# jrl-umi3218/jrl-walkgen

Measured on AMD Instinct MI355X. Metric: QP-MPC ticks/sec (batch=4096, N=16), higher is better.
Workload: dtype f64

## Files before the change

### jrl-walkgen_amd/csrc/wg_capi.hip

```cpp
#include <hip/hip_runtime.h>

#include <climits>
#include <cmath>
#include <cstdarg>
#include <cstdio>
#include <cstdlib>
#include <cstring>
#include <limits>
#include <memory>
#include <mutex>
#include <string>
#include <type_traits>
#include <vector>

#include "../../include/wg_mpc.h"
#include "wg_ql_device.hpp"
#include "wg_tick_device.hpp"
#include "wg_tick_kernels.hpp"
#include "wg_pldp_device.hpp"
#include "wg_dimitrov_device.hpp"
#include "wg_preview_device.hpp"
#include "wg_gramian_device.hpp"
#include "wg_zmpdisc_device.hpp"
#include "wg_footcons_device.hpp"
// ... 562 lines not shown
  m->hip_l_lo = -30.0 / 180.0 * wg::kPi; m->hip_l_hi = 45.0 / 180.0 * wg::kPi;
  m->hip_r_lo = -30.0 / 180.0 * wg::kPi; m->hip_r_hi = 45.0 / 180.0 * wg::kPi;
  m->hip_vmax = 0.0; m->hip_amax = 0.1; m->feet_cross_max = 5.0 / 180.0 * wg::kPi;
  m->step_period = 0.8; m->ds_period = 1e9; m->dsss_period = 0.8;
  m->t_single = 0.7; m->t_double = 0.1; m->step_height = 0.05; m->feet_distance = 0.2;
}

void wg_gait_init(const wg_model_t *, wg_gait_state_t *s, const double com0[3], const double left_xyt[3],
                  const double right_xyt[3]) {
  memset(s, 0, sizeof *s);
  s->online = 1; s->time_to_stop = -1.0;
  for (int k = 0; k < 3; k++) {
    s->lf[k].x = left_xyt[0]; s->lf[k].y = left_xyt[1]; s->lf[k].theta = left_xyt[2];
    s->rf[k].x = right_xyt[0]; s->rf[k].y = right_xyt[1]; s->rf[k].theta = right_xyt[2];
  }
  s->phase = WG_DS; s->foot = WG_LEFT; s->time_limit = 1000000000; s->nb_steps_left = 1;
  s->sup_x = left_xyt[0]; s->sup_y = left_xyt[1]; s->sup_yaw = left_xyt[2] * wg::kPi / 180;
  s->com_x[0] = com0[0]; s->com_y[0] = com0[1]; s->com_z = com0[2];
  s->front_com_x[0] = com0[0]; s->front_com_y[0] = com0[1];
  s->nb_steps_ssds = 2; s->rot_support_foot = WG_LEFT;
}

int wg_mpc_configure_ctx(wg_ctx_t *ctx, const wg_model_t *model) {
  if (int rc = use_ctx(ctx)) return rc;
  if (!model) return fail(WG_ERR_BAD_ARG, "null model");
  if (model->N < 2 || model->N > wg::kNMaxH) return fail(WG_ERR_BAD_ARG, "N=%d outside [2,%d]", model->N, wg::kNMaxH);
  if ((int)(model->T / model->Tctrl) != WG_SAMPLES_PER_TICK)
    return fail(WG_ERR_BAD_ARG, "T/Tctrl must be %d", WG_SAMPLES_PER_TICK);
  if (tick_max_prw_steps(*model) > wg::kSMax)
    return fail(WG_ERR_BAD_ARG, "step_period=%g: a horizon of N=%d instants of T=%g previews up to %d steps, the tick holds %d",
                model->step_period, model->N, model->T, tick_max_prw_steps(*model), wg::kSMax);
  const size_t lds = TickPlan(*model).lds;
  if (lds > 160 * 1024) return fail(WG_ERR_TOO_LARGE, "tick needs %zu B of LDS > 160 KiB", lds);
  std::vector<double> qb;
  if (model->flags & (WG_FLAG_GRAMIAN_MFMA_F64 | WG_FLAG_GRAMIAN_MFMA_F32)) {
    qb.resize((size_t)model->N * model->N);
    const int prec = (model->flags & WG_FLAG_GRAMIAN_MFMA_F32) ? WG_GRAMIAN_F32 : WG_GRAMIAN_F64;
    if (int rc = wg_gramian_batch_ctx(ctx, 1, model->N, &model->T, &model->com_height_qp, model->alpha, model->beta, model->gamma,
                                  prec, qb.data()))
      return rc;
  }
  std::lock_guard<std::mutex> lk(ctx->mu);
  std::unique_ptr<wg::TickTables> host_tables_p(new wg::TickTables);
  wg::TickTables &host_tables = *host_tables_p;
  wg::build_tables(*model, host_tables, qb.empty() ? nullptr : qb.data());
  if (!host_tables.blocks_ok && !qb.empty())
    return fail(WG_ERR_BAD_ARG, "the matrix-core Gramian is not positive definite enough for ql0002's factorisation");
  if (const char *e = getenv("WG_QL_SUMS")) {
    const std::string v(e);
    if (v == "ordered") host_tables.ql_sums = wg::kSumsOrdered;
    else if (v == "doubt") host_tables.ql_sums = wg::kSumsDoubt;
    else if (!v.empty() && v != "guarded") return fail(WG_ERR_BAD_ARG, "WG_QL_SUMS=%s: ordered, doubt or unset", e);
  }
  if (!ctx->tables_dev) HIP_TRY(hipMalloc(reinterpret_cast<void **>(&ctx->tables_dev), sizeof(wg::TickTables)));
  if (!ctx->model_dev) HIP_TRY(hipMalloc(reinterpret_cast<void **>(&ctx->model_dev), sizeof(wg_model_t)));
  if (int rc = ctx_wait_own(ctx)) return rc;
  HostScope hs(ctx);
  WG_H2D(ctx->tables_dev, &host_tables, sizeof host_tables);
  WG_H2D(ctx->model_dev, model, sizeof(wg_model_t));
  WG_HOST_WAIT();
  ctx->model = *model;
  ctx->model_set = true;
  return WG_OK;
}

size_t wg_mpc_tick_lds_bytes_for(const wg_model_t *model) {
  if (!model || model->N < 2 || model->N > wg::kNMaxH || tick_max_prw_steps(*model) > wg::kSMax) return 0;
  return TickPlan(*model).lds;
}

size_t wg_mpc_tick_lds_bytes_ctx(wg_ctx_t *ctx) {
  if (!ctx || !ctx->model_set) return 0;
  return TickPlan(ctx->model).lds;
}

int wg_mpc_reserve_ctx(wg_ctx_t *ctx, int max_gaits) {
  if (int rc = use_ctx(ctx)) return rc;
  if (!ctx->model_set) return fail(WG_ERR_BAD_ARG, "wg_mpc_configure() has not been called on this context");
  if (max_gaits < 1) return fail(WG_ERR_BAD_ARG, "max_gaits = %d", max_gaits);
  const TickPlan plan(ctx->model);
  std::lock_guard<std::mutex> launch_lk(ctx->launch_mu);
  double *zs = nullptr;
  if (int rc = plan.reserve_slots(ctx, max_gaits, &zs)) return rc;
  return ctx->run_buf.reserve(run_buf_bytes(max_gaits));
}

}
namespace {
int tick_launch(wg_ctx_t *ctx, int B, wg_gait_state_t *states, wg_tick_out_t *outs, int *diag, int advance_calls, int *hist, int hist_cap, int *hist_len, void *hip_stream, wg_gait_state_t *host_states, int *host_done) {
  if (int rc = tick_check(ctx, B, states)) return rc;
  if (hist && (!hist_len || hist_cap <= 0)) return fail(WG_ERR_BAD_ARG, "hist needs hist_len and hist_cap > 0");
  if (B == 0) return WG_OK;
  const TickPlan plan(ctx->model);
  if (int rc = plan.raise_lds(WG_KERNEL_BY_VIEW(wg_mpc_tick_kernel, plan.view))) return rc;
  const int grid = B;
  hipStream_t st = reinterpret_cast<hipStream_t>(hip_stream);
  std::lock_guard<std::mutex> launch_lk(ctx->launch_mu);
  if (int rc = slot_claim(ctx, ctx->guard_order, st, "tick / run")) return rc;
  double *zs = nullptr;
  if (int rc = plan.reserve_slots(ctx, grid, &zs)) return rc;
  int *order = nullptr, *iters_out = nullptr;
  if (B > ctx->num_cu * plan.per_cu() && !host_states && env_flag("WG_TICK_LPT", true))
    if (int rc = lpt_prepare(ctx->tick_lpt, states, B, st, &order, &iters_out)) return rc;
  WG_LAUNCH_BY_VIEW(wg_mpc_tick_kernel, plan.view, grid, plan.launch_lds, st, B, ctx->model, ctx->tables_dev, states, outs, diag, advance_calls, hist,
                    hist_cap, hist_len, (unsigned)plan.qlb, zs, (unsigned)plan.zslot, plan.ecap, host_states, host_done, order, iters_out);
  HIP_TRY(hipGetLastError());
// ... 1350 lines not shown
```

### jrl-walkgen_amd/csrc/wg_prof.hpp

```cpp
#pragma once
#include <hip/hip_runtime.h>

namespace wg {

enum ProfSlot : int {
  PS_NORMS = 0, PS_DIAGCHK = 1, PS_CHOL = 2 , PS_INVERSE = 3,
  PS_RESID = 4, PS_ZTWW_RESID = 5, PS_XSHIFT = 6, PS_BACKSUB_RESID = 7, PS_XMAG_RESID = 8,
  PS_SCAN = 9, PS_FDIFF = 10, PS_NEWNORMAL = 11, PS_SWEEP = 12, PS_ROUTE = 13, PS_STEP_PRE = 14, PS_BACKSUB_STEP = 15,
  PS_PICKDROP = 16, PS_STEP = 17, PS_ADD = 18, PS_XMAG_ADD = 19, PS_TAIL = 20,
  PS_RESET_BODY = 24, PS_RESID_GRAD = 25, PS_RESID_FWD = 26, PS_RESID_GX = 27,
  PS_N_ROUTE = 28, PS_N_COORD = 29, PS_N_DEPENDENT = 30, PS_BORDER_ROWS = 31,
  PS_SW_NORMS = 32, PS_SW_COEFF = 33, PS_SW_ROWS = 34,
  PS_TICK_PRE = 21, PS_TICK_ASSEMBLY = 22, PS_TICK_POST = 23,
  PS_TICK_LOAD = 35, PS_TICK_FSM = 36, PS_TICK_ORIENT = 37, PS_TICK_INSTANTS = 38,
  PS_TICK_COM = 39, PS_TICK_TRUNK = 40, PS_TICK_FEET = 41, PS_TICK_QUEUE = 42,
  PS_N_FALLBACK = 43, PS_N_RERUN = 44,
  PS_COUNT = 48
};

#ifdef WG_PROFILE
__device__ unsigned long long g_prof[PS_COUNT];

struct PtState {
  unsigned long long acc[28] = {0}, cnt[4] = {0}, sw[3] = {0}, cnt2[2] = {0};
  unsigned long long last = clock64();
};
#define PT_DECL PtState pt;
#define PT_PARAM , PtState &pt
#define PT_ARG , pt
#define PT(k) do { unsigned long long t_ = clock64(); pt.acc[k] += t_ - pt.last; pt.last = t_; } while (0)
#define PT_VIA(k, mem, reg) do { mem = reg; PT(k); reg = mem; } while (0)
#define PT_FLUSH do { if ((threadIdx.x & 63) == 0) { for (int k_ = 0; k_ < 28; ++k_) if (k_ < PS_TICK_PRE || k_ > PS_TICK_POST) atomicAdd(&g_prof[k_], pt.acc[k_]); \
                                                      for (int k_ = 0; k_ < 4; ++k_) atomicAdd(&g_prof[PS_N_ROUTE + k_], pt.cnt[k_]); \
                                                      for (int k_ = 0; k_ < 3; ++k_) atomicAdd(&g_prof[PS_SW_NORMS + k_], pt.sw[k_]); \
                                                      for (int k_ = 0; k_ < 2; ++k_) atomicAdd(&g_prof[PS_N_FALLBACK + k_], pt.cnt2[k_]); } } while (0)
#define PT_SW_PARAM , unsigned long long *ptsw = nullptr
#define PT_SW_ARG , pt.sw
#define PT_SW(k) do { if (ptsw) { unsigned long long t_ = clock64(); ptsw[(k) - PS_SW_NORMS] += t_ - ptsw_last; ptsw_last = t_; } } while (0)
#define PT_SW_BEGIN unsigned long long ptsw_last = clock64();
#define PT_COUNT(k) do { pt.cnt[(k) - PS_N_ROUTE]++; } while (0)
#define PT_COUNT2(k) do { pt.cnt2[(k) - PS_N_FALLBACK]++; } while (0)
#define PT_LOCAL_BEGIN unsigned long long ptl_last = clock64();
#define PT_LOCAL(k) do { unsigned long long t_ = clock64(); if ((threadIdx.x & 63) == 0) atomicAdd(&g_prof[k], t_ - ptl_last); ptl_last = t_; } while (0)

struct TkState {
  unsigned long long acc[PS_COUNT] = {0};
  unsigned long long last = clock64();
};
#define TK_DECL TkState tk;
#define TK(k) do { unsigned long long t_ = clock64(); tk.acc[k] += t_ - tk.last; tk.last = t_; } while (0)
#define TK_RESTART do { tk.last = clock64(); } while (0)
#define TK_ADD_(k) atomicAdd(&g_prof[k], tk.acc[k])
#define TK_FLUSH do { if ((threadIdx.x & 63) == 0) { const unsigned long long store_ = clock64() - tk.last; \
    TK_ADD_(PS_TICK_LOAD); TK_ADD_(PS_TICK_FSM); TK_ADD_(PS_TICK_ORIENT); TK_ADD_(PS_TICK_INSTANTS); TK_ADD_(PS_TICK_ASSEMBLY); \
    TK_ADD_(PS_TICK_COM); TK_ADD_(PS_TICK_TRUNK); TK_ADD_(PS_TICK_FEET); TK_ADD_(PS_TICK_QUEUE); \
    atomicAdd(&g_prof[PS_TICK_PRE], tk.acc[PS_TICK_LOAD] + tk.acc[PS_TICK_FSM] + tk.acc[PS_TICK_ORIENT] + tk.acc[PS_TICK_INSTANTS]); \
    atomicAdd(&g_prof[PS_TICK_POST], tk.acc[PS_TICK_COM] + tk.acc[PS_TICK_TRUNK] + tk.acc[PS_TICK_FEET] + tk.acc[PS_TICK_QUEUE] + store_); } } while (0)
#else
#define PT_DECL
#define PT_PARAM
#define PT_ARG
#define PT(k) do {} while (0)
#define PT_VIA(k, mem, reg) ((void)0)
#define PT_FLUSH do {} while (0)
#define PT_SW_PARAM
#define PT_SW_ARG
#define PT_SW(k) do {} while (0)
#define PT_SW_BEGIN
#define PT_COUNT(k) do {} while (0)
#define PT_COUNT2(k) do {} while (0)
#define PT_LOCAL_BEGIN
#define PT_LOCAL(k) ((void)0)
#define TK_DECL
#define TK(k) ((void)0)
#define TK_RESTART ((void)0)
#define TK_FLUSH ((void)0)
#endif

}
```

### jrl-walkgen_amd/csrc/wg_ql_device.hpp

```cpp
#pragma once
#include <hip/hip_runtime.h>

#include <type_traits>

#include "wg_wave.hpp"
#include "wg_ql_view.hpp"
#include "wg_ql_phases.hpp"
#define WG_GUARD_FN __device__ __forceinline__
#define WG_GUARD_K(c) ::wg::wg_kconst(c)
#include "wg_ql_guard.hpp"

namespace wg {

#define WG_BACKSUB(q, s, nact, lane)                                                                   \
  do {                                                                                                 \
    if constexpr (P::kNM > 0 && P::kNM + 12 <= 48) backsub_lds<48>(q, s, nact, lane, q.sc0);          \
    else if (P::kNM == 0 && (P::kWideN || q.n >= 48) && (nact) <= 60) backsub_lds<96>(q, s, nact, lane, q.sc0);     \
    else if (P::kNM == 0 && !P::kRowOps && q.n >= 24 && (nact) <= 36) backsub_lds<48>(q, s, nact, lane, q.sc0); \
    else backsub(q, s, nact, lane);                                                                    \
  } while (0)
#define WG_SWEEP(q, s, nu, nact, lane) \
  do { if (P::kNM > 0 || (!P::kRowOps && q.n <= 64)) sweep_flat<P::kFixedLdz>(q, s, nu, nact, lane PT_SW_ARG); else sweep<(P::kRowOps ? WG_ELEM_GRP : 8), P::kWideN>(q, s, nu, nact, lane); } while (0)

#define QL_SCAN_ACCEPT                                                                        \
  if (wak <= 0.0) continue;                                                                   \
  double sumx = -sum * wak;                                                                   \
  if (k + 1 <= me) sumx = fabs(sumx);                                                         \
  if (sumx <= 0.0) continue;                                                                  \
  if (bidx >= 0 && sumx <= bestv) continue;                                                   \
  double tempa = temp + fabs(sum);                                                            \
  if (tempa <= temp) continue;                                                                \
  temp += onha * fabs(sum);                                                                   \
  if (temp <= tempa) continue;                                                                \
  bestv = sumx; bestres = sum; bestw = wak; bidx = k + 1
template <class P>
__device__ __forceinline__ QlResult ql_solve(const QlView &q, P &prob, double vsmall, int *hist, int hist_cap, QlResume *rs = nullptr) {
  constexpr bool kNan = P::kNanExact && (WG_NAN_REGIME != 0);
  constexpr bool kGuard = GuardedSumsOf<P>::value;
  [[maybe_unused]] int gmode = kSumsOrdered;
  if constexpr (kGuard) gmode = uni(prob.sums_mode);
  int lane = wg_lane();
  const int n = q.n, m = q.m, me = q.me, mn = q.mn;
  QlResult out;
  out.hist_len = 0;
  const bool resuming = rs != nullptr && rs->valid != 0;
  int nact = 0, info = 0, iterc = 1, itref = 0, iflag = 0;
  const int maxit = (m + n) * 40;
  const double onha = 1.5, xmagr = .01, diagr = 2.0;
  const int ifinc = 3, kfinc = n > 10 ? n : 10;
  int jfinc = -kfinc;
  double xmag = 0.0, vfact = 1.0, res = 0.0, ratio = 0.0, diag = 0.0;
  double wsel = 1.0;
  int knext = 0;
  const int s_tail = q.r_tail;
  double *s = q.R + s_tail;
  bool early_exit = false;
  bool cap_hit = false;
  bool x_suspect = false;
  auto x_has_non_numbers = [&]() {
    bool b = false;
    for (int i = lane; i < n; i += 64) { const bool bi = !wg_sane(q.x[i]); b = b || bi; }
    return __ballot(b) != 0ull;
  };
  PT_DECL
  if (resuming) {
    nact = rs->nact; info = rs->info; iterc = rs->iterc; itref = rs->itref; iflag = rs->iflag; jfinc = rs->jfinc; knext = rs->knext;
    out.hist_len = rs->hist_len;
    xmag = rs->xmag; vfact = rs->vfact; res = rs->res; ratio = rs->ratio; diag = rs->diag;
    if constexpr (kNan) x_suspect = x_has_non_numbers();
  }

#define LOG_EVENT(code)                                                   \
  do {                                                                    \
    if (lane == 0 && hist && out.hist_len < hist_cap) hist[out.hist_len] = (code); \
    out.hist_len++;                                                       \
  } while (0)
#define QL_RERUN_ORDERED                                                              \
  do {                                                                                \
    PT_COUNT2(PS_N_RERUN);                                                            \
    for (int i = lane; i < n; i += 64) prob.setGd(q, i, q.wd[i]);                     \
    WG_WSYNC();                                                                       \
    PT_FLUSH;                                                                         \
    out.ifail = kQlDoubt; out.n_iter = iterc; out.nact = nact;                        \
    return out;                                                                       \
  } while (0)

  if (!resuming) {
    int fatal = 0x7fffffff;
    if constexpr (P::kCompact) {
      fatal = prob.norms(q, lane);
    } else {
      for (int k = lane; k < m; k += 64) {
        double sum = 0.0;
// ... 771 lines not shown
          reset = verdict == kGuardReset;
        }
        if (reset) st = ST_RESET;
        else if (itref <= 0) st = ST_SCAN;
        else st = ST_RESID;
      } else {
      WG_REP(6) { sm = uni(xmag_sum(q, prob, vfact, lane)); WG_SINK(sm); }
      xmag = maxd(xmag, sm);
      PT(PS_XMAG_ADD);
      if (WG_UBOOL(sm < wg_kconst(xmagr) * xmag)) st = ST_RESET;
      else if (itref <= 0) st = ST_SCAN;
      else st = ST_RESID;
      }
      if (q.nact_cap > 0 && nact > q.nact_cap) { cap_hit = true; break; }
      if (st == ST_SCAN) goto next_scan;
      continue;
    }

    if (st == ST_CONVERGED) {
      ++itref;
      jfinc = -1;
      if (itref == 1) { st = ST_RESID; continue; }
      st = ST_FINISH;
    }
  }
  if constexpr (kGuard) { if (gmode == kSumsDoubt && !early_exit && !cap_hit) QL_RERUN_ORDERED; }
#undef QL_RERUN_ORDERED
#undef LOG_EVENT

  PT(PS_TAIL);
  PT_FLUSH;
  if (cap_hit) {
    if (rs) {
      rs->nact = nact; rs->info = info; rs->iterc = iterc; rs->itref = itref; rs->iflag = iflag; rs->jfinc = jfinc; rs->knext = knext;
      rs->st = st; rs->hist_len = out.hist_len;
      rs->xmag = xmag; rs->vfact = vfact; rs->res = res; rs->ratio = ratio; rs->diag = diag;
    }
    out.ifail = kQlCapHit; out.n_iter = iterc; out.nact = nact;
    return out;
  }
  out.ifail = ql_ifail_of(info);
  out.n_iter = iterc;
  out.nact = nact;
  return out;
}

template <class P>
__device__ __forceinline__ QlResult ql_solve_guarded(const QlView &q, P &prob, double vsmall, int *hist, int hist_cap) {
  static_assert(GuardedSumsOf<P>::value, "for policies with kGuardedSums");
  QlResult r;
  for (;;) {
    r = ql_solve(q, prob, vsmall, hist, hist_cap);
    if (!WG_UBOOL(r.ifail == kQlDoubt)) break;
    prob.sums_mode = kSumsOrdered;
  }
  return r;
}

}
```

### jrl-walkgen_amd/csrc/wg_ql_herdt.hpp

```cpp
#pragma once
#include "wg_ql_device.hpp"

namespace wg {

constexpr int kSMaxQ = 4;
constexpr int kGvLd = 4;
constexpr int kQbLd = 32;

template <int NH, int NS>
__device__ __forceinline__ bool herdt_border_rows(const QlView &q, const double *gd, const double *Gv, double vsmall, int lane) {
  constexpr int M2 = 2 * NH;
  const int i = lane;
  const bool jerk = i < NH, foot = i >= NH && i < NH + NS, row = jerk || foot;
  const int fi = i - NH;
  const int gi = jerk ? i : M2 + (foot ? fi : 0);
  double acc[NS];
#pragma unroll
  for (int f = 0; f < NS; ++f)
    acc[f] = (jerk || (foot && f >= fi)) ? ((foot && f == fi) ? gd[gi] : Gv[gi * kGvLd + f]) : 0.0;
  const double dreg = jerk ? Rf(i, i) : 1.0;
  const int colbase = jerk ? i * (i + 1) / 2 : 0;
  const int khi = jerk ? i : 0;
  double rnext = (0 < khi) ? q.Rf[colbase] : 0.0;
  for (int k = 0; k < NH; ++k) {
// ... 123 lines not shown
    }
    for (int e = lane; e < NH * NH; e += 64) { const int i = e % NH, j = NH + e / NH; Rf(i, j) = 0.0; }
    for (int e = lane; e < NH * NH; e += 64) {
      const int i = e % NH, j = e / NH;
      const double v = Z2[i + j * M2];
      Zm(i, j) = v; Zm(NH + i, NH + j) = v;
      Zm(NH + i, j) = 0.0;
      Zm(i, NH + j) = ((z2sign[e >> 6] >> (e & 63)) & 1ull) ? wg_kconst(-0.0) : 0.0;
    }
    for (int e = lane; e < (n - M2) * M2; e += 64) { const int i = M2 + e % (n - M2), j = e / (n - M2); Zm(i, j) = 0.0; }
    return;
  }
  double rv[TR], zv[TZ];
#pragma unroll
  for (int t = 0; t < TR; ++t) { const int e = lane + 64 * t; rv[t] = e < NR ? R2[e] : 0.0; }
#pragma unroll
  for (int t = 0; t < TZ; ++t) { const int e = lane + 64 * t; zv[t] = e < NH * NH ? Z2[(e % NH) + (e / NH) * M2] : 0.0; }
#pragma unroll
  for (int t = 0; t < TR; ++t) {
    const int e = lane + 64 * t;
    if (e < NR) {
      int j = 0;
      while ((j + 1) * (j + 2) / 2 <= e) ++j;
      const int i = e - j * (j + 1) / 2;
      q.Rf[e] = rv[t];
      Rf(NH + i, NH + j) = rv[t];
    }
  }
  for (int e = lane; e < NH * NH; e += 64) { const int i = e % NH, j = NH + e / NH; Rf(i, j) = 0.0; }
#pragma unroll
  for (int t = 0; t < TZ; ++t) {
    const int e = lane + 64 * t;
    if (e < NH * NH) {
      const int i = e % NH, j = e / NH;
      Zm(i, j) = zv[t]; Zm(NH + i, NH + j) = zv[t];
      Zm(NH + i, j) = 0.0;
      Zm(i, NH + j) = ((z2sign[e >> 6] >> (e & 63)) & 1ull) ? wg_kconst(-0.0) : 0.0;
    }
  }
  for (int e = lane; e < (n - M2) * M2; e += 64) { const int i = M2 + e % (n - M2), j = e / (n - M2); Zm(i, j) = 0.0; }
}

template <int NH>
struct HerdtProb {
  static constexpr bool kCompact = true;
  static constexpr bool kNanExact = WG_TICK_NAN_EXACT != 0;
  static constexpr bool kHasFactor = true;
  static constexpr bool kRowOps = false;
  static constexpr int kNM = 2 * NH + 2 * 2;
  static constexpr int kCopRows = 4 * NH;
  static constexpr bool kWideN = false;
  static constexpr int kFixedLdz = kNM | 1;
  static constexpr bool kGuardedSums = true;
  static_assert(4 * NH == 64, "one CoP row per lane needs 4N == 64");
  const double *Qb;
  const double *u;
  double *Gv;
  double *gd;
  const double *rowA, *rowB;
  const int *rowK, *stepidx;
  const double *V_f;
  const double *R2, *Z2;
  const unsigned long long *z2sign;
  double diag_b;
  int blocks_ok;
  int ns;
  int sums_mode;
  double ax[NH], ay[NH];
  int fj;
  double ra, rb;
  double bcop;
  double ga, gb; int gk;
  __device__ __forceinline__ double fa() const { return ra + 0.0; }
  __device__ __forceinline__ double fb() const { return rb + 0.0; }
  struct FootRow { double v[4]; int c[4]; };
  __device__ __forceinline__ FootRow foot_row() const {
    const bool used = gk >= 0, pred = gk > 0;
    const int kk = used ? gk : 0;
    FootRow r;
    const int c1 = 2 * NH + kk, c3 = 2 * NH + ns + kk;
    r.c[0] = used ? (pred ? c1 - 1 : c1) : 2 * NH; r.c[1] = used ? c1 : 2 * NH;
    r.c[2] = used ? (pred ? c3 - 1 : c3) : 2 * NH; r.c[3] = used ? c3 : 2 * NH;
    r.v[0] = pred ? ga + 0.0 : 0.0; r.v[1] = used ? 0.0 - ga : 0.0;
    r.v[2] = pred ? gb + 0.0 : 0.0; r.v[3] = used ? 0.0 - gb : 0.0;
    return r;
  }

  __device__ __forceinline__ double G(const QlView &q, int i, int j) const {
    if (i == j) return gd[i];
    if (j < i) { const int t = i; i = j; j = t; }
    if (j < 2 * NH) {
      if (i < NH && j < NH) return Qb[i * kQbLd + j];
      if (i >= NH && j >= NH) return Qb[(i - NH) * kQbLd + (j - NH)];
      return 0.0;
    }
    return Gv[i * kGvLd + (j - 2 * NH)];
  }
  __device__ __forceinline__ double Gd(const QlView &, int i) const { return gd[i]; }
  __device__ __forceinline__ void setGd(const QlView &, int i, double v) const { gd[i] = v; }
  __device__ __forceinline__ double xl(const QlView &, int) const { return -1e8; }
  __device__ __forceinline__ double xu(const QlView &, int) const { return 1e8; }

  __device__ __forceinline__ double A(const QlView &, int k, int i) const {
    k = uni(k);
    if (k == 0) return 0.0;
    const bool cop = k <= 4 * NH;
// ... 495 lines not shown
```

### jrl-walkgen_amd/csrc/wg_ql_phases.hpp

```cpp
#pragma once
#include <hip/hip_runtime.h>

#include <type_traits>

#include "wg_wave.hpp"
#include "wg_ql_view.hpp"

namespace wg {

#ifndef WG_ELEM_GRP
#define WG_ELEM_GRP 4
#endif

__device__ __forceinline__ double sqrt_1to2(double x) {
  const double y = __builtin_amdgcn_rsq(x);
  double g = x * y;
  double h = y * 0.5;
  const double r = __builtin_fma(-h, g, 0.5);
  g = __builtin_fma(g, r, g);
  h = __builtin_fma(h, r, h);
  double d = __builtin_fma(-g, g, x);
  g = __builtin_fma(d, h, g);
  d = __builtin_fma(-g, g, x);
  g = __builtin_fma(d, h, g);
  return g;
}
__device__ __forceinline__ double givens_norm(double p, double qq) {
  const double ap = fabs(p), aq = fabs(qq);
  const bool pbig = ap >= aq;
  double t;
  asm("v_max_f64 %0, |%1|, |%2|" : "=v"(t) : "v"(p), "v"(qq));
  const double d = (pbig ? qq : p) / t;
  const double x = 1.0 + d * d;
  return t * sqrt_1to2(x);
}
__device__ __forceinline__ double givens_norm_fast(double p, double qq) {
  double t, a;
  asm("v_max_f64 %0, |%1|, |%2|" : "=v"(t) : "v"(p), "v"(qq));
  asm("v_min_f64 %0, |%1|, |%2|" : "=v"(a) : "v"(p), "v"(qq));
  double r = __builtin_amdgcn_rcp(t);
  double e = __builtin_fma(-t, r, 1.0);
  r = __builtin_fma(r, e, r);
  e = __builtin_fma(-t, r, 1.0);
  r = __builtin_fma(r, e, r);
  const double q0 = a * r;
  const double rem = __builtin_fma(-t, q0, a);
  const double d = __builtin_fma(rem, r, q0);
  const double x = 1.0 + d * d;
  return t * sqrt_1to2(x);
}
template <bool kOnePass = false>
__device__ __forceinline__ bool sweep_range_ok(const double *s, int lo, int hi, int lane) {
  if constexpr (kOnePass) {
    const int j = lo + lane;
    const bool in = j < hi;
    const double v = fabs(s[in ? j : lo]);
    return __ballot(in && !(v == 0.0 || (v >= 0x1p-400 && v <= 0x1p400))) == 0ull;
  }
  bool bad = false;
  for (int j = lo + lane; j < hi; j += 64) {
    const double v = fabs(s[j]);
    bad = bad || !(v == 0.0 || (v >= 0x1p-400 && v <= 0x1p400));
  }
  return __ballot(bad) == 0ull;
}
__device__ __forceinline__ void givens(double p, double qq, double &ga, double &gb, double &nrm) {
  const double sum = givens_norm(p, qq);
  ga = p / sum;
  gb = qq / sum;
  nrm = sum;
}
__device__ __forceinline__ bool significant(double base, double delta_abs) {
  double temp = base + delta_abs * wg_kconst(.1);
  double tempa = base + delta_abs * wg_kconst(.2);
  if (temp <= base) return false;
  if (tempa <= temp) return false;
  return true;
}

template <int NM = 0, int GRP = 8, bool kWide = false>
__device__ __forceinline__ void zt_times_ww(const QlView &q, double *s, int lane) {
  const int n = q.n;
  if (kWide || ((NM == 0 || NM > 64) && n > 64 && n <= 128)) {
    const int i0 = lane, i1 = lane + 64 < n ? lane + 64 : 0;
    const double *z0 = q.Z + (size_t)i0 * q.ldz, *z1 = q.Z + (size_t)i1 * q.ldz;
    double a0 = 0.0, a1 = 0.0;
    int j = 0;
    for (; j + GRP <= n; j += GRP) {
      double u0[GRP], u1[GRP], w[GRP];
#pragma unroll
      for (int e = 0; e < GRP; ++e) { u0[e] = *(z0 + j + e); u1[e] = *(z1 + j + e); w[e] = q.ww[j + e]; }
#pragma unroll
      for (int e = 0; e < GRP; ++e) { a0 += u0[e] * w[e]; a1 += u1[e] * w[e]; }
    }
    for (; j < n; ++j) { const double w = q.ww[j]; a0 += z0[j] * w; a1 += z1[j] * w; }
    s[i0] = a0;
    if (lane + 64 < n) s[i1] = a1;
    WG_WSYNC();
    return;
  }
  for (int i = lane; i < n; i += 64) {
    double acc = 0.0;
    WG_UNROLL
// ... 232 lines not shown
    for (; j >= 1; j -= 2) { bs_row<kBsLen>(q, buf, j, S, A9, B9); bs_row<kBsLen>(q, buf, j - 1, S, B9, A9); }
    if (j == 0) bs_row<kBsLen>(q, buf, 0, S, A9, B9);
  }
  if constexpr (kBsLen <= 64) {
    if (nact > 0) {
      const double wl = rl(S.w, nact - 1);
      q.ww[S.mine ? lane : nact - 1] = S.mine ? S.w : wl;
    }
  } else if (S.mine) q.ww[lane] = S.w;
  WG_WSYNC();
}


#ifndef WG_OS_CHUNK
#define WG_OS_CHUNK 12
#endif
constexpr int kOsChunk = WG_OS_CHUNK;
template <int NM>
__device__ __forceinline__ double ordered_sum_lds(double term, double *scratch, int cnt, int lane) {
  {
    const double v = (lane < cnt) ? term : 0.0;
    const double vl = rl(v, NM - 1);
    scratch[lane < NM ? lane : NM - 1] = lane < NM ? v : vl;
  }
  WG_WSYNC();
  double sum = 0.0;
#pragma unroll
  for (int i0 = 0; i0 < NM; i0 += kOsChunk) {
    double t[kOsChunk];
#pragma unroll
    for (int i = 0; i < kOsChunk; ++i) t[i] = (i0 + i < NM) ? scratch[i0 + i] : 0.0;
#pragma unroll
    for (int i = 0; i < kOsChunk; ++i) if (i0 + i < NM) sum += t[i];
  }
  WG_WSYNC();
  return sum;
}

template <int NM>
__device__ __forceinline__ double ordered_sum_lds_rolled(double term, double *scratch, int cnt, int lane) {
  {
    const double v = (lane < cnt) ? term : 0.0;
    const double vl = rl(v, NM - 1);
    scratch[lane < NM ? lane : NM - 1] = lane < NM ? v : vl;
  }
  WG_WSYNC();
  double sum = 0.0;
#pragma nounroll
  for (int i = 0; i < NM; ++i) sum += scratch[i];
  WG_WSYNC();
  return sum;
}

template <int kLdzC = 0>
__device__ __forceinline__ void sweep_flat(const QlView &q, double *s, int nu, int nact, int lane PT_SW_PARAM) {
  const int n = q.n;
  if (nu - 1 <= nact) return;
  PT_SW_BEGIN
  double *chain = q.sc2;
  WG_REP(3)
  if (sweep_range_ok<true>(s, nact, nu, lane)) {
    double cur = s[nu - 1];
    double pa = s[nu - 2], pb;
    int c = nu - 1;
    typedef __attribute__((address_space(3))) double lds_f64;
    const lds_f64 *sp = (const lds_f64 *)(s + (nu - 4));
    lds_f64 *cp = (lds_f64 *)(chain + (nu - 3));
    asm volatile("" : "+v"(sp), "+v"(cp));
    const int rots = c - nact;
    if (WG_UBOOL(cur != 0.0)) {
      for (int k = rots >> 1; k > 0; --k) {
        pb = sp[1];
        cur = givens_norm_fast(pa, cur); cp[1] = cur;
        pa = sp[0];
        cur = givens_norm_fast(pb, cur); cp[0] = cur;
        sp -= 2; cp -= 2;
      }
      if (rots & 1) { cur = givens_norm_fast(pa, cur); cp[1] = cur; }
    } else {
      for (int k = rots >> 1; k > 0; --k) {
        pb = sp[1];
        { const double nrmc = givens_norm_fast(pa, cur); cur = (cur == 0.0) ? pa : nrmc; cp[1] = cur; }
        pa = sp[0];
        { const double nrmc = givens_norm_fast(pb, cur); cur = (cur == 0.0) ? pb : nrmc; cp[0] = cur; }
        sp -= 2; cp -= 2;
      }
      if (rots & 1) { const double nrmc = givens_norm_fast(pa, cur); cur = (cur == 0.0) ? pa : nrmc; cp[1] = cur; }
    }
  } else {
    double cur = s[nu - 1];
    double p = s[nu - 2];
    for (int c = nu - 1; c > nact; --c) {
      const int nx = (c - 2 >= 0) ? c - 2 : 0;
      const double p_next = s[nx];
      const double nrmc = givens_norm(p, cur);
      cur = (cur == 0.0) ? p : nrmc;
      chain[c - 1] = cur;
      p = p_next;
    }
  }
  WG_WSYNC();
  PT_SW(PS_SW_NORMS);
  double myP = 0.0, myQ = 0.0, myN = 0.0;
  {
    const bool mine = lane > nact && lane < nu;
    const int c = mine ? lane : nu - 1;
    myP = s[c - 1];
    myQ = (c == nu - 1) ? s[nu - 1] : chain[c];
    const double chl = chain[c - 1];
    myN = (myQ == 0.0) ? 0.0 : chl;
  }
  WG_WSYNC();
  double *gab = q.sc0;
  bool any_skip;
  {
    const bool mine = lane > nact && lane < nu;
    const bool rot = mine && myN != 0.0;
    const double den = rot ? myN : 1.0;
    const double ga = rot ? myP / den : 2.0;
    const double gb = rot ? myQ / den : 0.0;
    any_skip = __ballot(mine && !rot) != 0ull;
    const int cl = mine ? lane : nu - 1;
    const double ga_l = rl(ga, nu - 1), gb_l = rl(gb, nu - 1);
    const double ga_w = mine ? ga : ga_l, gb_w = mine ? gb : gb_l;
    gab[2 * cl] = ga_w; gab[2 * cl + 1] = gb_w;
    if (rot) s[lane - 1] = myN;
  }
  WG_WSYNC();
  PT_SW(PS_SW_COEFF);
  {
    const int i = lane < n ? lane : n - 1;
    const int ldz = q.ldz;
    double *zp = q.Z + i + (nu - 1) * ldz;
    double carry = zp[0];
    struct Op { double zl, ga, gb; };
    auto fetch = [&](int c) -> Op {
      const int cc = c > nact ? c : nact + 1;
      Op o; o.zl = q.Z[i + (cc - 1) * ldz]; o.ga = gab[2 * cc]; o.gb = gab[2 * cc + 1];
      return o;
    };
    auto rotate = [&](const Op &o) {
      const bool skip = (o.ga == 2.0);
      const double t_r = o.ga * o.zl + o.gb * carry;
      const double z_r = o.ga * carry - o.gb * o.zl;
      zp[0] = skip ? carry : z_r;
      carry = skip ? o.zl : t_r;
      zp -= ldz;
    };
    auto rotate_all = [&](const Op &o) {
      const double t_r = o.ga * o.zl + o.gb * carry;
      zp[0] = o.ga * carry - o.gb * o.zl;
      carry = t_r;
      zp -= ldz;
    };
    Op s0 = fetch(nu - 1), s1 = fetch(nu - 2), s2 = fetch(nu - 3);
    int c = nu - 1;
    if (any_skip) {
// ... 690 lines not shown
```

### jrl-walkgen_amd/csrc/wg_ql_view.hpp

```cpp
#pragma once
#include <hip/hip_runtime.h>

#include <type_traits>

#include "wg_wave.hpp"
#include "wg_prof.hpp"

namespace wg {

struct QlDims {
  int n, m, mmax;
  int ldg, ldz, lda;
  bool dense;
  bool a_lds;
  int nsc;
  bool bounds;
  bool z_lds;
  bool wab_lds;
  bool cold_lds;
  int r_cols;
  bool g_lds;
  __host__ __device__ QlDims(int n_, int m_, int mmax_, bool dense_ = true, bool a_lds_ = true, int nsc_ = 0,
                             bool bounds_ = true, bool z_lds_ = true, bool wab_lds_ = true, bool cold_lds_ = true, int r_cols_ = 0,
                             bool g_lds_ = true)
// ... 115 lines not shown
  static constexpr bool kNanExact = true;
  static constexpr bool kHasFactor = false;
  static constexpr bool kRowOps = false;
  static constexpr int kNM = kNMc;
  static constexpr bool kWideN = false;
  static constexpr int kFixedLdz = kNMc > 0 ? (kNMc | 1) : 0;
  __device__ __forceinline__ double G(const QlView &q, int i, int j) const;
  __device__ __forceinline__ double A(const QlView &q, int k, int i) const;
  __device__ __forceinline__ double Gd(const QlView &q, int i) const;
  __device__ __forceinline__ void setGd(const QlView &q, int i, double v) const;
  __device__ __forceinline__ double xl(const QlView &q, int i) const;
  __device__ __forceinline__ double xu(const QlView &q, int i) const;
};
typedef DenseProbT<true> DenseProb;
template <int NM, int MM>
struct DenseRegProb : DenseProbT<false, NM> {
  static constexpr bool kRegRows = true;
  double ar0[NM], ar1[NM];
  __device__ __forceinline__ void load_rows(const QlView &q, int lane) {
    const int m = q.m;
    const int mc = m > 0 ? m - 1 : 0;
    const int k0 = lane < m ? lane : mc, k1 = lane + 64 < m ? lane + 64 : mc;
#pragma unroll
    for (int i = 0; i < NM; ++i) { ar0[i] = q.A[k0 + i * q.lda]; ar1[i] = q.A[k1 + i * q.lda]; }
  }
  __device__ __forceinline__ void row_to(const QlView &q, int k, double *dst, int lane) const {
    const int n = q.n;
    if (lane == (k & 63)) {
#pragma unroll
      for (int i = 0; i < NM; ++i)
        if (i < n) dst[i] = k < 64 ? ar0[i] : ar1[i];
    }
  }
};
template <class P, class = void> struct HasRegRows { static constexpr bool value = false; };
template <class P> struct HasRegRows<P, typename std::enable_if<P::kRegRows>::type> { static constexpr bool value = true; };
#define Rp(i, j) q.R[(j) * ((j) + 1) / 2 + (i)]
#define Rf(i, j) q.Rf[(j) * ((j) + 1) / 2 + (i)]

#ifdef WG_REPEAT_PHASE
#define WG_REP(id) for (int wg_rep_ = 0; wg_rep_ < (((WG_REPEAT_PHASE) == (id)) ? 2 : 1); ++wg_rep_, ({ asm volatile("" ::: "memory"); }))
#define WG_SINK(x) asm volatile("" ::"v"(x))
#else
#define WG_REP(id)
#define WG_SINK(x) do {} while (0)
#endif

struct NoActiveParams {};
template <class P, class = void> struct ActiveParamsOf { typedef NoActiveParams type; };
template <class P> struct ActiveParamsOf<P, typename std::enable_if<P::kCompact>::type> { typedef typename P::ActiveParams type; };

template <class P, class = void> struct GuardedSumsOf { static constexpr bool value = false; };
template <class P> struct GuardedSumsOf<P, typename std::enable_if<P::kGuardedSums>::type> { static constexpr bool value = true; };
enum : int { kSumsGuarded = 0, kSumsOrdered = 1, kSumsDoubt = 2 };
constexpr int kQlDoubt = -7778;

struct QlResult {
  int ifail, n_iter, nact, hist_len;
};
struct QlResume {
  int valid = 0;
  int nact, info, iterc, itref, iflag, jfinc, knext, st, hist_len;
  double xmag, vfact, res, ratio, diag;
};

template <bool kGLds, int kNMc> __device__ __forceinline__ double DenseProbT<kGLds, kNMc>::G(const QlView &q, int i, int j) const {
  if constexpr (kGLds) return q.G[i + j * q.ldg];
  else {
    const double g = q.G[i + j * q.ldg], dg = q.Gdiag[i];
    return i == j ? dg : g;
  }
}
template <bool kGLds, int kNMc> __device__ __forceinline__ double DenseProbT<kGLds, kNMc>::A(const QlView &q, int k, int i) const { return q.A[k + i * q.lda]; }
template <bool kGLds, int kNMc> __device__ __forceinline__ double DenseProbT<kGLds, kNMc>::Gd(const QlView &q, int i) const {
  if constexpr (kGLds) return q.G[i + i * q.ldg]; else return q.Gdiag[i];
}
template <bool kGLds, int kNMc> __device__ __forceinline__ void DenseProbT<kGLds, kNMc>::setGd(const QlView &q, int i, double v) const {
  if constexpr (kGLds) q.G[i + i * q.ldg] = v; else q.Gdiag[i] = v;
}
template <bool kGLds, int kNMc> __device__ __forceinline__ double DenseProbT<kGLds, kNMc>::xl(const QlView &q, int i) const { return q.xl[i]; }
template <bool kGLds, int kNMc> __device__ __forceinline__ double DenseProbT<kGLds, kNMc>::xu(const QlView &q, int i) const { return q.xu[i]; }

}
```

### jrl-walkgen_amd/csrc/wg_wave.hpp

```cpp
#pragma once
#include <hip/hip_runtime.h>

namespace wg {

#ifndef WG_UNROLL_N
#define WG_UNROLL_N 4
#endif
#define WG_PRAGMA(x) _Pragma(#x)
#define WG_UNROLL_(n) WG_PRAGMA(unroll n)
#define WG_UNROLL WG_UNROLL_(WG_UNROLL_N)

#define WG_WSYNC()                                          \
  do {                                                      \
    __builtin_amdgcn_fence(__ATOMIC_RELEASE, "wavefront");  \
    __builtin_amdgcn_wave_barrier();                        \
    __builtin_amdgcn_fence(__ATOMIC_ACQUIRE, "wavefront");  \
  } while (0)

__device__ __forceinline__ int wg_lane() { int l = threadIdx.x & 63; asm volatile("" : "+v"(l)); return l; }
__device__ __forceinline__ int uni(int v) { return __builtin_amdgcn_readfirstlane(v); }
__device__ __forceinline__ double uni(double v) {
  int lo = __double2loint(v), hi = __double2hiint(v);
  lo = __builtin_amdgcn_readfirstlane(lo);
  hi = __builtin_amdgcn_readfirstlane(hi);
// ... 22 lines not shown
}
__device__ __forceinline__ double maxd(double a, double b) { return a >= b ? a : b; }
__device__ __forceinline__ double mind(double a, double b) { return a <= b ? a : b; }

template <int CTRL>
__device__ __forceinline__ int dpp_keep(int v) { return __builtin_amdgcn_update_dpp(v, v, CTRL, 0xf, 0xf, false); }
template <int CTRL>
__device__ __forceinline__ double dpp_keep(double v) {
  const int lo = dpp_keep<CTRL>(__double2loint(v)), hi = dpp_keep<CTRL>(__double2hiint(v));
  return __hiloint2double(hi, lo);
}
__device__ __forceinline__ double wave_max(double v) {
  v = __builtin_fmax(v, dpp_keep<0x111>(v));
  v = __builtin_fmax(v, dpp_keep<0x112>(v));
  v = __builtin_fmax(v, dpp_keep<0x114>(v));
  v = __builtin_fmax(v, dpp_keep<0x118>(v));
  v = __builtin_fmax(v, dpp_keep<0x142>(v));
  v = __builtin_fmax(v, dpp_keep<0x143>(v));
  return rl(v, 63);
}
__device__ __forceinline__ int wave_min_int(int v) {
  { const int o = dpp_keep<0x111>(v); v = o < v ? o : v; }
  { const int o = dpp_keep<0x112>(v); v = o < v ? o : v; }
  { const int o = dpp_keep<0x114>(v); v = o < v ? o : v; }
  { const int o = dpp_keep<0x118>(v); v = o < v ? o : v; }
  { const int o = dpp_keep<0x142>(v); v = o < v ? o : v; }
  { const int o = dpp_keep<0x143>(v); v = o < v ? o : v; }
  return __builtin_amdgcn_readlane(v, 63);
}
__device__ __forceinline__ int wave_max_int(int v) {
  { const int o = dpp_keep<0x111>(v); v = o > v ? o : v; }
  { const int o = dpp_keep<0x112>(v); v = o > v ? o : v; }
  { const int o = dpp_keep<0x114>(v); v = o > v ? o : v; }
  { const int o = dpp_keep<0x118>(v); v = o > v ? o : v; }
  { const int o = dpp_keep<0x142>(v); v = o > v ? o : v; }
  { const int o = dpp_keep<0x143>(v); v = o > v ? o : v; }
  return __builtin_amdgcn_readlane(v, 63);
}
template <int CTRL, int ROWS>
__device__ __forceinline__ double dpp_zero(double v) {
  const int lo = __builtin_amdgcn_update_dpp(0, __double2loint(v), CTRL, ROWS, 0xf, true);
  const int hi = __builtin_amdgcn_update_dpp(0, __double2hiint(v), CTRL, ROWS, 0xf, true);
  return __hiloint2double(hi, lo);
}
__device__ __forceinline__ double wave_sum_tree(double v) {
  v += dpp_zero<0x111, 0xf>(v);
  v += dpp_zero<0x112, 0xf>(v);
  v += dpp_zero<0x114, 0xf>(v);
  v += dpp_zero<0x118, 0xf>(v);
  v += dpp_zero<0x142, 0xa>(v);
  v += dpp_zero<0x143, 0xc>(v);
  return rl(v, 63);
}
__device__ __forceinline__ void wave_argmax_first(double &v, int &idx) {
  const double vv = idx >= 0 ? v : -__builtin_huge_val();
  const double vmax = wave_max(vv);
  const int key = (idx >= 0 && v == vmax) ? idx : 0x7fffffff;
  const int kmin = wave_min_int(key);
  v = vmax;
  idx = kmin == 0x7fffffff ? -1 : kmin;
}

}
```

Baseline: 6.923 million.

## Seed Givens sweep norms with a parallel prefix-sum rsqrt chain

Adds a seeded path for the flat Givens sweep in the Herdt QL solver. Each lane computes a reciprocal-sqrt seed from a wave prefix sum of squared entries, so the serial chain of rotation norms needs only FMA refinement steps instead of divide and sqrt. The recorded norms are checked bit-exactly against the exact formula, with a fallback to the original serial sweep when any lane disagrees. This is meant to shorten the latency of the serial norm chain, at the cost of extra LDS traffic, two wave syncs and a verification pass, and any mismatch pays for both paths.

```diff
diff --git a/jrl-walkgen_amd/csrc/wg_capi.hip b/jrl-walkgen_amd/csrc/wg_capi.hip
--- a/jrl-walkgen_amd/csrc/wg_capi.hip
+++ b/jrl-walkgen_amd/csrc/wg_capi.hip
@@ -638,6 +638,12 @@
     else if (v == "doubt") host_tables.ql_sums = wg::kSumsDoubt;
     else if (!v.empty() && v != "guarded") return fail(WG_ERR_BAD_ARG, "WG_QL_SUMS=%s: ordered, doubt or unset", e);
   }
+  if (const char *e = getenv("WG_QL_NORMS")) {
+    const std::string v(e);
+    if (v == "exact") host_tables.ql_sums |= wg::kNormsExact;
+    else if (v == "doubt") host_tables.ql_sums |= wg::kNormsDoubt;
+    else if (!v.empty() && v != "seeded") return fail(WG_ERR_BAD_ARG, "WG_QL_NORMS=%s: seeded, exact, doubt or unset", e);
+  }
   if (!ctx->tables_dev) HIP_TRY(hipMalloc(reinterpret_cast<void **>(&ctx->tables_dev), sizeof(wg::TickTables)));
   if (!ctx->model_dev) HIP_TRY(hipMalloc(reinterpret_cast<void **>(&ctx->model_dev), sizeof(wg_model_t)));
   if (int rc = ctx_wait_own(ctx)) return rc;
diff --git a/jrl-walkgen_amd/csrc/wg_prof.hpp b/jrl-walkgen_amd/csrc/wg_prof.hpp
--- a/jrl-walkgen_amd/csrc/wg_prof.hpp
+++ b/jrl-walkgen_amd/csrc/wg_prof.hpp
@@ -15,6 +15,7 @@
   PS_TICK_LOAD = 35, PS_TICK_FSM = 36, PS_TICK_ORIENT = 37, PS_TICK_INSTANTS = 38,
   PS_TICK_COM = 39, PS_TICK_TRUNK = 40, PS_TICK_FEET = 41, PS_TICK_QUEUE = 42,
   PS_N_FALLBACK = 43, PS_N_RERUN = 44,
+  PS_N_SWEEPS = 45, PS_N_SEEDED = 46, PS_N_SEED_FALLBACK = 47,
   PS_COUNT = 48
 };
 
@@ -22,7 +23,7 @@
 __device__ unsigned long long g_prof[PS_COUNT];
 
 struct PtState {
-  unsigned long long acc[28] = {0}, cnt[4] = {0}, sw[3] = {0}, cnt2[2] = {0};
+  unsigned long long acc[28] = {0}, cnt[4] = {0}, sw[6] = {0}, cnt2[2] = {0};
   unsigned long long last = clock64();
 };
 #define PT_DECL PtState pt;
@@ -33,11 +34,13 @@
 #define PT_FLUSH do { if ((threadIdx.x & 63) == 0) { for (int k_ = 0; k_ < 28; ++k_) if (k_ < PS_TICK_PRE || k_ > PS_TICK_POST) atomicAdd(&g_prof[k_], pt.acc[k_]); \
                                                       for (int k_ = 0; k_ < 4; ++k_) atomicAdd(&g_prof[PS_N_ROUTE + k_], pt.cnt[k_]); \
                                                       for (int k_ = 0; k_ < 3; ++k_) atomicAdd(&g_prof[PS_SW_NORMS + k_], pt.sw[k_]); \
-                                                      for (int k_ = 0; k_ < 2; ++k_) atomicAdd(&g_prof[PS_N_FALLBACK + k_], pt.cnt2[k_]); } } while (0)
+                                                      for (int k_ = 0; k_ < 2; ++k_) atomicAdd(&g_prof[PS_N_FALLBACK + k_], pt.cnt2[k_]); \
+                                                      for (int k_ = 0; k_ < 3; ++k_) atomicAdd(&g_prof[PS_N_SWEEPS + k_], pt.sw[3 + k_]); } } while (0)
 #define PT_SW_PARAM , unsigned long long *ptsw = nullptr
 #define PT_SW_ARG , pt.sw
 #define PT_SW(k) do { if (ptsw) { unsigned long long t_ = clock64(); ptsw[(k) - PS_SW_NORMS] += t_ - ptsw_last; ptsw_last = t_; } } while (0)
 #define PT_SW_BEGIN unsigned long long ptsw_last = clock64();
+#define PT_SW_COUNT(k) do { if (ptsw) ptsw[3 + (k) - PS_N_SWEEPS]++; } while (0)
 #define PT_COUNT(k) do { pt.cnt[(k) - PS_N_ROUTE]++; } while (0)
 #define PT_COUNT2(k) do { pt.cnt2[(k) - PS_N_FALLBACK]++; } while (0)
 #define PT_LOCAL_BEGIN unsigned long long ptl_last = clock64();
@@ -67,6 +70,7 @@
 #define PT_SW_ARG
 #define PT_SW(k) do {} while (0)
 #define PT_SW_BEGIN
+#define PT_SW_COUNT(k) do {} while (0)
 #define PT_COUNT(k) do {} while (0)
 #define PT_COUNT2(k) do {} while (0)
 #define PT_LOCAL_BEGIN
diff --git a/jrl-walkgen_amd/csrc/wg_ql_device.hpp b/jrl-walkgen_amd/csrc/wg_ql_device.hpp
--- a/jrl-walkgen_amd/csrc/wg_ql_device.hpp
+++ b/jrl-walkgen_amd/csrc/wg_ql_device.hpp
@@ -20,7 +20,7 @@
     else backsub(q, s, nact, lane);                                                                    \
   } while (0)
 #define WG_SWEEP(q, s, nu, nact, lane) \
-  do { if (P::kNM > 0 || (!P::kRowOps && q.n <= 64)) sweep_flat<P::kFixedLdz>(q, s, nu, nact, lane PT_SW_ARG); else sweep<(P::kRowOps ? WG_ELEM_GRP : 8), P::kWideN>(q, s, nu, nact, lane); } while (0)
+  do { if (P::kNM > 0 || (!P::kRowOps && q.n <= 64)) sweep_flat<P::kFixedLdz, SeededNormsOf<P>::value>(q, s, nu, nact, lane, nmode PT_SW_ARG); else sweep<(P::kRowOps ? WG_ELEM_GRP : 8), P::kWideN>(q, s, nu, nact, lane); } while (0)
 
 #define QL_SCAN_ACCEPT                                                                        \
   if (wak <= 0.0) continue;                                                                   \
@@ -38,7 +38,9 @@
   constexpr bool kNan = P::kNanExact && (WG_NAN_REGIME != 0);
   constexpr bool kGuard = GuardedSumsOf<P>::value;
   [[maybe_unused]] int gmode = kSumsOrdered;
-  if constexpr (kGuard) gmode = uni(prob.sums_mode);
+  if constexpr (kGuard) gmode = uni(prob.sums_mode) & kSumsMask;
+  [[maybe_unused]] int nmode = kNormsExact;
+  if constexpr (SeededNormsOf<P>::value) nmode = uni(prob.sums_mode) & kNormsMask;
   int lane = wg_lane();
   const int n = q.n, m = q.m, me = q.me, mn = q.mn;
   QlResult out;
@@ -916,7 +918,7 @@
   for (;;) {
     r = ql_solve(q, prob, vsmall, hist, hist_cap);
     if (!WG_UBOOL(r.ifail == kQlDoubt)) break;
-    prob.sums_mode = kSumsOrdered;
+    prob.sums_mode = (prob.sums_mode & ~kSumsMask) | kSumsOrdered;
   }
   return r;
 }
diff --git a/jrl-walkgen_amd/csrc/wg_ql_herdt.hpp b/jrl-walkgen_amd/csrc/wg_ql_herdt.hpp
--- a/jrl-walkgen_amd/csrc/wg_ql_herdt.hpp
+++ b/jrl-walkgen_amd/csrc/wg_ql_herdt.hpp
@@ -199,6 +199,7 @@
   static constexpr bool kWideN = false;
   static constexpr int kFixedLdz = kNM | 1;
   static constexpr bool kGuardedSums = true;
+  static constexpr bool kSeededNorms = true;
   static_assert(4 * NH == 64, "one CoP row per lane needs 4N == 64");
   const double *Qb;
   const double *u;
diff --git a/jrl-walkgen_amd/csrc/wg_ql_norms.hpp b/jrl-walkgen_amd/csrc/wg_ql_norms.hpp
--- /dev/null
+++ b/jrl-walkgen_amd/csrc/wg_ql_norms.hpp
@@ -0,0 +1,81 @@
+#pragma once
+#include <cmath>
+
+#ifndef WG_NORMS_FN
+#define WG_NORMS_FN inline
+#endif
+#ifndef WG_NORMS_RSQ
+#define WG_NORMS_RSQ(x) (1.0 / std::sqrt(x))
+#endif
+
+namespace wg {
+
+struct NormSeed { double r, y; };
+
+WG_NORMS_FN double norms_rsqrt(double v) {
+  double y = WG_NORMS_RSQ(v);
+  {
+    const double g = v * y, h = 0.5 * y;
+    const double e = __builtin_fma(-h, g, 0.5);
+    y = __builtin_fma(y, e, y);
+  }
+  {
+    const double g = v * y, h = 0.5 * y;
+    const double e = __builtin_fma(-h, g, 0.5);
+    y = __builtin_fma(y, e, y);
+  }
+  return y;
+}
+
+WG_NORMS_FN NormSeed norms_seed(double p2, double s2) {
+  const bool pbig = p2 >= s2;
+  const double t2 = pbig ? p2 : s2, a2 = pbig ? s2 : p2;
+  NormSeed o;
+  o.r = norms_rsqrt(t2);
+  const double x = 1.0 + a2 * (o.r * o.r);
+  o.y = norms_rsqrt(x);
+  return o;
+}
+
+WG_NORMS_FN double norms_step(double t, double a, double r, double y) {
+  const double q0 = a * r;
+  const double rem = __builtin_fma(-t, q0, a);
+  const double d = __builtin_fma(rem, r, q0);
+  const double x = 1.0 + d * d;
+  const double yh = 0.5 * y;
+  const double g0 = x * y;
+  const double e = __builtin_fma(-g0, g0, x);
+  const double g = __builtin_fma(e, yh, g0);
+  return t * g;
+}
+
+#ifndef WG_NORMS_EXACT
+inline double norms_exact(double p, double q) {
+  const double ap = std::fabs(p), aq = std::fabs(q);
+  const double t = ap >= aq ? ap : aq, a = ap >= aq ? aq : ap;
+  const double d = a / t;
+  return t * std::sqrt(1.0 + d * d);
+}
+#define WG_NORMS_EXACT(p, q) ::wg::norms_exact(p, q)
+#endif
+
+WG_NORMS_FN bool norms_same_bits(double a, double b) {
+  unsigned long long x, y;
+  __builtin_memcpy(&x, &a, sizeof x);
+  __builtin_memcpy(&y, &b, sizeof y);
+  return x == y;
+}
+WG_NORMS_FN bool norms_rotation_ok(double p, double q, double recorded) {
+  const double want = (q == 0.0) ? p : WG_NORMS_EXACT(p, q);
+  return norms_same_bits(want, recorded);
+}
+
+inline void norms_prefix_scan(double *v ) {
+  for (int w = 1; w < 16; w *= 2)
+    for (int i = 63; i >= 0; --i) if ((i & 15) >= w) v[i] = v[i] + v[i - w];
+  for (int i = 16; i < 32; ++i) v[i] = v[i] + v[15];
+  for (int i = 48; i < 64; ++i) v[i] = v[i] + v[47];
+  for (int i = 32; i < 64; ++i) v[i] = v[i] + v[31];
+}
+
+}
diff --git a/jrl-walkgen_amd/csrc/wg_ql_phases.hpp b/jrl-walkgen_amd/csrc/wg_ql_phases.hpp
--- a/jrl-walkgen_amd/csrc/wg_ql_phases.hpp
+++ b/jrl-walkgen_amd/csrc/wg_ql_phases.hpp
@@ -49,6 +49,12 @@
   const double x = 1.0 + d * d;
   return t * sqrt_1to2(x);
 }
+}
+#define WG_NORMS_FN __device__ __forceinline__
+#define WG_NORMS_RSQ(x) __builtin_amdgcn_rsq(x)
+#define WG_NORMS_EXACT(p, q) ::wg::givens_norm_fast(p, q)
+#include "wg_ql_norms.hpp"
+namespace wg {
 template <bool kOnePass = false>
 __device__ __forceinline__ bool sweep_range_ok(const double *s, int lo, int hi, int lane) {
   if constexpr (kOnePass) {
@@ -387,13 +393,74 @@
   return sum;
 }
 
-template <int kLdzC = 0>
-__device__ __forceinline__ void sweep_flat(const QlView &q, double *s, int nu, int nact, int lane PT_SW_PARAM) {
+template <int kLdzC = 0, bool kSeeded = false>
+__device__ __forceinline__ void sweep_flat(const QlView &q, double *s, int nu, int nact, int lane, [[maybe_unused]] int nmode = kNormsExact PT_SW_PARAM) {
   const int n = q.n;
   if (nu - 1 <= nact) return;
   PT_SW_BEGIN
+  PT_SW_COUNT(PS_N_SWEEPS);
   double *chain = q.sc2;
-  WG_REP(3)
+  [[maybe_unused]] bool seeded_ok = false;
+  [[maybe_unused]] double sdP = 0.0, sdQ = 0.0, sdN = 0.0;
+  WG_REP(3) {
+  if constexpr (kSeeded) {
+    seeded_ok = false;
+    if (nmode != kNormsExact && sweep_range_ok<true>(s, nact, nu, lane)) {
+      PT_SW_COUNT(PS_N_SEEDED);
+      typedef __attribute__((address_space(3))) double lds_f64;
+      double *seeds = q.sc0;
+      int top;
+      {
+        const int j = nu - 1 - lane;
+        const bool in = j >= nact;
+        const double sj = s[in ? j : nact], pj = s[j > nact ? j - 1 : nact];
+        const unsigned long long nz = __ballot(in && j > nact && sj != 0.0);
+        top = nz ? nu - __builtin_ctzll(nz) : nact + 1;
+        if (in && j >= top - 1 && j < nu - 1) chain[j] = sj;
+        const double s2 = wave_prefix_sum(in ? sj * sj : 0.0);
+        const NormSeed sd = norms_seed(pj * pj, s2);
+        if (j > nact && j < top) { seeds[2 * j] = sd.r; seeds[2 * j + 1] = sd.y; }
+      }
+      WG_WSYNC();
+      const int rots = top - 1 - nact;
+      if (rots > 0) {
+        double cur = s[top - 1];
+        double pa = s[top - 2], pb;
+        const lds_f64 *sp = (const lds_f64 *)(s + (top - 4));
+        lds_f64 *cp = (lds_f64 *)(chain + (top - 3));
+        const lds_f64 *dp = (const lds_f64 *)(seeds + 2 * (top - 3));
+        asm volatile("" : "+v"(sp), "+v"(cp), "+v"(dp));
+        double ra = dp[4], ya = dp[5], rb, yb;
+        auto step = [](double p, double cur_in, double r, double y) -> double {
+          double t, a;
+          asm("v_max_f64 %0, |%1|, |%2|" : "=v"(t) : "v"(p), "v"(cur_in));
+          asm("v_min_f64 %0, |%1|, |%2|" : "=v"(a) : "v"(p), "v"(cur_in));
+          return norms_step(t, a, r, y);
+        };
+        for (int k = rots >> 1; k > 0; --k) {
+          pb = sp[1]; rb = dp[2]; yb = dp[3];
+          cur = step(pa, cur, ra, ya); cp[1] = cur;
+          pa = sp[0]; ra = dp[0]; ya = dp[1];
+          cur = step(pb, cur, rb, yb); cp[0] = cur;
+          sp -= 2; cp -= 2; dp -= 4;
+        }
+        if (rots & 1) { cur = step(pa, cur, ra, ya); cp[1] = cur; }
+      }
+      WG_WSYNC();
+      {
+        const bool mine = lane > nact && lane < nu;
+        const int c = mine ? lane : nu - 1;
+        sdP = s[c - 1];
+        sdQ = (c == nu - 1) ? s[nu - 1] : chain[c];
+        sdN = chain[c - 1];
+        const bool bad = !norms_rotation_ok(sdP, sdQ, sdN);
+        seeded_ok = (__ballot(bad) == 0ull) && nmode != kNormsDoubt;
+      }
+      if (!seeded_ok) PT_SW_COUNT(PS_N_SEED_FALLBACK);
+    }
+  }
+  if (kSeeded && seeded_ok) {
+  } else
   if (sweep_range_ok<true>(s, nact, nu, lane)) {
     double cur = s[nu - 1];
     double pa = s[nu - 2], pb;
@@ -434,10 +501,13 @@
       p = p_next;
     }
   }
+  }
   WG_WSYNC();
   PT_SW(PS_SW_NORMS);
   double myP = 0.0, myQ = 0.0, myN = 0.0;
-  {
+  if (kSeeded && seeded_ok) {
+    myP = sdP; myQ = sdQ; myN = (sdQ == 0.0) ? 0.0 : sdN;
+  } else {
     const bool mine = lane > nact && lane < nu;
     const int c = mine ? lane : nu - 1;
     myP = s[c - 1];
diff --git a/jrl-walkgen_amd/csrc/wg_ql_view.hpp b/jrl-walkgen_amd/csrc/wg_ql_view.hpp
--- a/jrl-walkgen_amd/csrc/wg_ql_view.hpp
+++ b/jrl-walkgen_amd/csrc/wg_ql_view.hpp
@@ -191,7 +191,10 @@
 
 template <class P, class = void> struct GuardedSumsOf { static constexpr bool value = false; };
 template <class P> struct GuardedSumsOf<P, typename std::enable_if<P::kGuardedSums>::type> { static constexpr bool value = true; };
-enum : int { kSumsGuarded = 0, kSumsOrdered = 1, kSumsDoubt = 2 };
+enum : int { kSumsGuarded = 0, kSumsOrdered = 1, kSumsDoubt = 2, kSumsMask = 3 };
+template <class P, class = void> struct SeededNormsOf { static constexpr bool value = false; };
+template <class P> struct SeededNormsOf<P, typename std::enable_if<P::kSeededNorms>::type> { static constexpr bool value = true; };
+enum : int { kNormsSeeded = 0, kNormsExact = 1 << 8, kNormsDoubt = 2 << 8, kNormsMask = 3 << 8 };
 constexpr int kQlDoubt = -7778;
 
 struct QlResult {
diff --git a/jrl-walkgen_amd/csrc/wg_wave.hpp b/jrl-walkgen_amd/csrc/wg_wave.hpp
--- a/jrl-walkgen_amd/csrc/wg_wave.hpp
+++ b/jrl-walkgen_amd/csrc/wg_wave.hpp
@@ -98,6 +98,15 @@
   v += dpp_zero<0x143, 0xc>(v);
   return rl(v, 63);
 }
+__device__ __forceinline__ double wave_prefix_sum(double v) {
+  v += dpp_zero<0x111, 0xf>(v);
+  v += dpp_zero<0x112, 0xf>(v);
+  v += dpp_zero<0x114, 0xf>(v);
+  v += dpp_zero<0x118, 0xf>(v);
+  v += dpp_zero<0x142, 0xa>(v);
+  v += dpp_zero<0x143, 0xc>(v);
+  return v;
+}
 __device__ __forceinline__ void wave_argmax_first(double &v, int &idx) {
   const double vv = idx >= 0 ? v : -__builtin_huge_val();
   const double vmax = wave_max(vv);
```

Result: faster. 7.202 million, median of 6 (+4.0%).
